# TinfoilHat0/Defending-Against-Backdoors-with-Robust-Learning-Rate

Measured on NVIDIA H100. Metric: fl_rounds_per_sec, higher is better.
Workload: dtype bf16

## Files before the change

defending-against-backdoors-with-robust-learning-rate_b200/ops/csrc/conv_halo.cu:

```cuda
#include <cuda.h>

#include "common.cuh"
#include "gemm.h"
#include "wgmma.cuh"

namespace rlr {

using namespace wg;

cudaError_t make_tmap_bf16(CUtensorMap* map, const void* base, int rank, const uint64_t* dims, const uint64_t* strides_bytes,
                           const uint32_t* box, const uint32_t* elem_strides = nullptr);

constexpr int HL_THREADS = 256 + 32;
constexpr int HL_TH = 16, HL_TW = 8;
constexpr int HL_PITCH = 16;
constexpr int HL_HALO_BYTES = (HL_TH + 2) * HL_PITCH * 128;
constexpr int HL_W_BYTES = 9 * 64 * 128;
constexpr int HL_STAGES = 3;
constexpr int HL_PITCH_OUT = 64 * 2 + 16;
constexpr int HL_STAGING = 128 * HL_PITCH_OUT;
constexpr int HL_SMEM = HL_W_BYTES + HL_STAGES * HL_HALO_BYTES + 2 * HL_STAGING + 1024 + 1024;

struct HaloParams {
    int NB, H, W;
// ... 104 lines not shown
                    const uint64_t db = smem_desc_sw128(w_base + tp * 8192 + k * 32, 16, 1024);
#pragma unroll
                    for (int m = 0; m < 2; ++m) {
                        const uint32_t a0 = halo + (dy * HL_PITCH + dx) * 128 + m * 8 * HL_PITCH * 128 + k * 32;
                        const uint32_t bo = p.bo_mode ? ((a0 >> 7) & 7u) : 0u;
                        wgmma_bf16<64, 0, 0>(acc[m], smem_desc_sw128(a0, 16, HL_PITCH * 128, bo), db, (tp > 0 || k > 0) ? 1u : 0u);
                    }
                }
            }
            wgmma_commit();
            wgmma_wait<0>();
            fence_acc(acc[0]);
            fence_acc(acc[1]);
            if (lane == 0) mbar_arrive(&sh->halo_empty[stage]);
            if (trace) p.dbg[q * 8 + 3] = clock64();
#pragma unroll
            for (int m = 0; m < 2; ++m)
#pragma unroll
                for (int j = 0; j < 8; ++j) {
                    const int c = frag_col(t, 4 * j);
#pragma unroll
                    for (int h = 0; h < 2; ++h) {
                        float a = acc[m][4 * j + 2 * h], b = acc[m][4 * j + 2 * h + 1];
                        a += sh->bias[c]; b += sh->bias[c + 1];
                        if (p.relu) { a = fmaxf(a, 0.f); b = fmaxf(b, 0.f); }
                        const uint32_t packed = pack_bf16x2(a, b);
                        if (kStats) {
                            const float2 rq = __bfloat1622float2(*reinterpret_cast<const __nv_bfloat162*>(&packed));
                            st1[2 * j] += rq.x; st1[2 * j + 1] += rq.y;
                            st2[2 * j] += rq.x * rq.x; st2[2 * j + 1] += rq.y * rq.y;
                        }
                        *reinterpret_cast<uint32_t*>(stage_buf + (m * 64 + r0 + 8 * h) * HL_PITCH_OUT + c * 2) = packed;
                    }
                }
            named_bar(1 + wgi, 128);
            if (trace) p.dbg[q * 8 + 6] = clock64();
#pragma unroll
            for (int it = 0; it < 8; ++it) {
                const int idx = t + it * 128;
                const int rr = idx >> 3, ch = idx & 7;
                if (col0 + ch * 8 >= p.N) continue;
                const int h = h0 + (rr >> 3), w = w0 + (rr & 7);
                if (h >= p.H || w >= p.W) continue;
                const size_t gi = ((size_t)n * p.H + h) * p.W + w;
                uint4 val = *reinterpret_cast<const uint4*>(stage_buf + rr * HL_PITCH_OUT + ch * 16);
                uint4* gp = reinterpret_cast<uint4*>(out + gi * p.ldc + col0 + ch * 8);
                if (kAcc) {
                    const __nv_bfloat162* o2 = reinterpret_cast<const __nv_bfloat162*>(&oldv[it]);
                    __nv_bfloat162* v2 = reinterpret_cast<__nv_bfloat162*>(&val);
#pragma unroll
                    for (int qq = 0; qq < 4; ++qq) {
                        const float2 a = __bfloat1622float2(v2[qq]), b = __bfloat1622float2(o2[qq]);
                        v2[qq] = __floats2bfloat162_rn(a.x + b.x, a.y + b.y);
                    }
                }
                *gp = val;
            }
            named_bar(1 + wgi, 128);
            if (trace) p.dbg[q * 8 + 7] = clock64();
        }
        if (kStats) {
#pragma unroll
            for (int i = 0; i < 16; ++i)
#pragma unroll
                for (int o = 4; o < 32; o <<= 1) {
                    st1[i] += __shfl_xor_sync(0xffffffffu, st1[i], o);
                    st2[i] += __shfl_xor_sync(0xffffffffu, st2[i], o);
                }
            if (lane < 4)
#pragma unroll
                for (int i = 0; i < 16; ++i) {
                    const int c = frag_col(t, 2 * (i & ~1)) + (i & 1);
                    atomicAdd(&sh->red[c], st1[i]);
                    atomicAdd(&sh->red[64 + c], st2[i]);
                }
            named_bar(3, 256);
            if (threadIdx.x < 128 && col0 + (threadIdx.x & 63) < p.N)
                atomicAdd(p.stats + (size_t)(blockIdx.x % kStatSlots) * 2 * p.N + (threadIdx.x < 64 ? 0 : p.N) + col0 + (threadIdx.x & 63),
                          sh->red[threadIdx.x]);
        }
    }
}

cudaError_t launch_conv3x3_halo_bf16(const void* x, const void* w, void* out, int NB, int Hin, int Win, int H, int W, int Cout, const float* bias,
                                     int relu, int accumulate, float* stats, int bo_mode, long long* dbg, int num_sms, cudaStream_t st) {
    const int pad = (H - Hin + 2) / 2;
    if (pad < 0 || pad > 2 || H != Hin + 2 * pad - 2 || W != Win + 2 * pad - 2 || H < 1 || W < 1 || Cout % 8) return cudaErrorInvalidValue;
    if (stats && (H % HL_TH || W % HL_TW)) return cudaErrorInvalidValue;
    static bool configured = false;
    if (!configured) {
        RLR_CUDA_CHECK(cudaFuncSetAttribute(umma_conv3x3_halo_kernel<false, false>, cudaFuncAttributeMaxDynamicSharedMemorySize, HL_SMEM));
        RLR_CUDA_CHECK(cudaFuncSetAttribute(umma_conv3x3_halo_kernel<true, false>, cudaFuncAttributeMaxDynamicSharedMemorySize, HL_SMEM));
        RLR_CUDA_CHECK(cudaFuncSetAttribute(umma_conv3x3_halo_kernel<false, true>, cudaFuncAttributeMaxDynamicSharedMemorySize, HL_SMEM));
        configured = true;
    }
    if (stats && accumulate) return cudaErrorInvalidValue;
    HaloParams p{};
    p.NB = NB; p.H = H; p.W = W; p.pad = pad;
    p.tiles_h = (H + HL_TH - 1) / HL_TH; p.tiles_w = (W + HL_TW - 1) / HL_TW; p.num_tiles = NB * p.tiles_h * p.tiles_w;
    p.N = Cout; p.out = out; p.ldc = Cout; p.bias = bias; p.stats = stats; p.relu = relu; p.accumulate = accumulate; p.bo_mode = bo_mode; p.dbg = dbg;
    CUtensorMap tmX, tmW;
    {
        const uint64_t d[4] = {64, (uint64_t)Win, (uint64_t)Hin, (uint64_t)NB};
        const uint64_t s[3] = {128, (uint64_t)Win * 128, (uint64_t)Hin * Win * 128};
        const uint32_t b[4] = {64, HL_PITCH, HL_TH + 2, 1};
        RLR_CUDA_CHECK(make_tmap_bf16(&tmX, x, 4, d, s, b));
    }
    {
        const uint64_t d[2] = {9 * 64, (uint64_t)Cout}, s[1] = {9 * 64 * 2};
        const uint32_t b[2] = {64, 64};
        RLR_CUDA_CHECK(make_tmap_bf16(&tmW, w, 2, d, s, b));
    }
    const int n_tiles_n = (Cout + 63) / 64;
    int gx = num_sms / n_tiles_n;
    if (gx > p.num_tiles) gx = p.num_tiles;
    if (gx < 1) gx = 1;
    const dim3 grid(gx, n_tiles_n);
    if (stats) return launch_kernel(umma_conv3x3_halo_kernel<true, false>, grid, dim3(HL_THREADS), HL_SMEM, st, tmX, tmW, p);
    if (accumulate) return launch_kernel(umma_conv3x3_halo_kernel<false, true>, grid, dim3(HL_THREADS), HL_SMEM, st, tmX, tmW, p);
    return launch_kernel(umma_conv3x3_halo_kernel<false, false>, grid, dim3(HL_THREADS), HL_SMEM, st, tmX, tmW, p);
}

}
```

defending-against-backdoors-with-robust-learning-rate_b200/ops/csrc/gemm.h:

```cpp
#pragma once
#include <cuda_runtime.h>
#include <cuda_bf16.h>
#include <stdint.h>

#include "dropspec.h"

namespace rlr {

constexpr int kStatSlots = 16;

struct ConvGemmParams {
    int M, N, num_kb;
    int mode;
    int cblocks;
    int TW, TH, TN;
    int Ho, Wo, NB;
    int tiles_w, tiles_h;
    int ntaps;
    int in_stride;
    int out_stride, out_ph, out_pw, OutH, OutW;
    int8_t dh[9], dw[9];
    int dn[9];
    int b_mn;
    int wtap[9];
    int wcols;
    DropSpec drop;
    int tma_store;
    int split_prod;
    long long* dbg;
    const __nv_bfloat16* b_src;
    int b_ld, b_kvalid;
    const uint32_t* wait_flags;
    int wait_lo, wait_hi;
    const uint32_t* wait_epoch;
    void* out;
    int ldc;
    const float* bias;
    float* stats;
    int stat_slots;
    int relu, accumulate;
};

cudaError_t launch_gemm_bf16(const void* A, const void* B, void* out, int M, int N, int K, int lda, int ldb, int ldc,
                             const float* bias, int relu, int accumulate, float* stats, cudaStream_t st, const DropSpec* drop = nullptr);
cudaError_t launch_stem_gemm_bf16(const void* A, const void* W, void* out, int M, int N, int kvalid, int ldw, const float* bias, int relu,
                                  float* stats, const uint32_t* wait_flags, int wait_lo, int wait_hi, const uint32_t* wait_epoch,
                                  cudaStream_t st);
void set_pdl(int on);
cudaError_t launch_gemm_splitk_bf16(const void* A, const void* B, void* out, float* ws, int M, int N, int K, const float* bias, int relu,
                                    int num_sms, cudaStream_t st, const DropSpec* drop = nullptr);
void set_persistent_conv(int on);
void set_conv_occ3(int level);
void set_conv_one_wave(int on);
void set_conv_tma_store(int on);
void set_conv_split_producer(int on);
void set_conv_trace(long long* buf);
long long* conv_trace_buf();
cudaError_t launch_conv_bf16(const void* x, const void* w, void* out, int NB, int planes, int Hin, int Win, int Cin, int Ho, int Wo,
                             int Cout, int ldc, int ntaps, const int* dh, const int* dw, const int* dplane, const float* bias,
                             int relu, int accumulate, float* stats, cudaStream_t st, const int* wtap = nullptr, int w_taps_total = 0,
                             int in_stride = 1, int out_stride = 1, int out_ph = 0, int out_pw = 0);

cudaError_t launch_conv3x3_halo_bf16(const void* x, const void* w, void* out, int NB, int Hin, int Win, int H, int W, int Cout, const float* bias,
                                     int relu, int accumulate, float* stats, int bo_mode, long long* dbg, int num_sms, cudaStream_t st);

cudaError_t launch_conv3x3_halo3_bf16(const void* x, const void* w, void* out, int NB, int H, int W, int Cout, const float* bias, int relu,
                                      int accumulate, int num_sms, cudaStream_t st);

cudaError_t launch_conv_wgrad_bf16(const void* dy, const void* x, float* dW, int NB, int planes, int Hin, int Win, int Cin, int Cin_valid,
                                   int Ho, int Wo, int Cout, int ntaps, const int* dh, const int* dw, const int* dplane, int num_sms,
                                   cudaStream_t st, int in_stride = 1);
cudaError_t launch_conv_wgrad_halo_bf16(const void* dy, const void* x, float* dW, int NB, int H, int W, int Cin_valid, int Cout,
                                        int num_sms, cudaStream_t st);
void set_wgrad_rows(int on);
void wgrad_launch_counts(long long* out);
cudaError_t launch_linear_wgrad_bf16(const void* dy, const void* x, float* dW, int B, int N, int K, int num_sms, cudaStream_t st);

cudaError_t launch_ordered_sum_f32(float* out, const float* part, int nparts, long long n, cudaStream_t st);
cudaError_t launch_ordered_sum_f64(double* out, const double* part, int nparts, long long n, cudaStream_t st);
cudaError_t launch_channel_stats(const __nv_bfloat16* x, long long M, int C, float* stats , int num_sms, cudaStream_t st,
                                 int only_sum = 0, int nslots = 1);
cudaError_t launch_bn_finalize(const float* stats, int slots, float* mean_rstd, float* running_mean, float* running_var, int C,
                               float count, float eps, float momentum, int train, cudaStream_t st);
cudaError_t launch_bn_apply(const __nv_bfloat16* x, const __nv_bfloat16* res, __nv_bfloat16* y, const float* gamma, const float* beta,
                            float* mean_rstd, long long M, int C, int relu, int fin_mode, const float* stats, int slots, float count,
                            float eps, float momentum, float* running_mean, float* running_var, int num_sms, cudaStream_t st);
cudaError_t launch_bn_bwd_reduce(const __nv_bfloat16* dy, const __nv_bfloat16* y, const __nv_bfloat16* x, const float* mean_rstd,
                                 float* dsum , long long M, int C, int relu, int num_sms, cudaStream_t st,
                                 const float* gamma = nullptr, const float* beta = nullptr, int nslots = 1);
cudaError_t launch_bn_bwd_apply(const __nv_bfloat16* dy, const __nv_bfloat16* y, const __nv_bfloat16* x, const float* gamma,
                                const float* mean_rstd, const float* dsum, __nv_bfloat16* dx, __nv_bfloat16* dres, float* dgamma,
                                float* dbeta, long long M, int C, int relu, int num_sms, cudaStream_t st, const float* beta = nullptr, int nslots = 1);
cudaError_t launch_gn_fwd(const __nv_bfloat16* x, const __nv_bfloat16* res, __nv_bfloat16* y, const float* gamma, const float* beta,
                          float* mean_rstd, int B, int HW, int C, int G, float eps, int relu, int num_sms, cudaStream_t st);
cudaError_t launch_gn_bwd(const __nv_bfloat16* dy, const __nv_bfloat16* y, const __nv_bfloat16* x, const float* gamma,
                          const float* mean_rstd, __nv_bfloat16* dx, __nv_bfloat16* dres, float* dgamma, float* dbeta, int B, int HW,
                          int C, int G, int relu, int num_sms, cudaStream_t st);
cudaError_t launch_relu_bwd(__nv_bfloat16* dy, const __nv_bfloat16* y, long long n, int num_sms, cudaStream_t st, float scale = 1.0f);
cudaError_t launch_maxpool2_fwd(const __nv_bfloat16* x, __nv_bfloat16* y, uint8_t* idx, int B, int H, int W, int C, cudaStream_t st,
                                float drop_p = 0.f, uint64_t seed = 0, const long long* step = nullptr, uint64_t stream = 0);
cudaError_t launch_maxpool2_bwd(const __nv_bfloat16* dy, const uint8_t* idx, __nv_bfloat16* dx, int B, int H, int W, int C, cudaStream_t st,
                                float drop_p, uint64_t seed, const long long* step, uint64_t stream, const __nv_bfloat16* zmask);
cudaError_t launch_avgpool_fwd(const __nv_bfloat16* x, __nv_bfloat16* y, int B, int HW, int C, cudaStream_t st);
cudaError_t launch_avgpool_bwd(const __nv_bfloat16* dy, __nv_bfloat16* dx, int B, int HW, int C, cudaStream_t st);
cudaError_t launch_dropout_fwd(const __nv_bfloat16* x, __nv_bfloat16* y, uint8_t* mask, long long n, float p, uint64_t seed,
                               const long long* step, uint64_t stream, cudaStream_t st);
cudaError_t launch_dropout_bwd(const __nv_bfloat16* dy, const uint8_t* mask, __nv_bfloat16* dx, long long n, float p, cudaStream_t st);
cudaError_t launch_space_to_depth(const __nv_bfloat16* x, __nv_bfloat16* y, int NB, int H, int W, int C, int num_sms, cudaStream_t st);
cudaError_t launch_im2col_small(const __nv_bfloat16* x, __nv_bfloat16* A, int NB, int H, int W, int C, int Ho, int Wo, int k, int pad,
                                int num_sms, cudaStream_t st);
cudaError_t launch_depth_to_space(const __nv_bfloat16* x4, __nv_bfloat16* y, int NB, int H, int W, int C, int accumulate, int plane_mask,
                                  int num_sms, cudaStream_t st);
cudaError_t launch_filter_gather_transpose(const __nv_bfloat16* w, __nv_bfloat16* wt, int Cout, int T, int Cin, int nsub, const int* taps,
                                           cudaStream_t st);
cudaError_t launch_filter_transpose(const __nv_bfloat16* w, __nv_bfloat16* wt, int Cout, int ntaps, int Cin, cudaStream_t st);
cudaError_t launch_linear_small_fwd(const __nv_bfloat16* x, const __nv_bfloat16* w, const float* bias, __nv_bfloat16* y, int B, int K,
                                    int N, int relu, cudaStream_t st);
cudaError_t launch_linear_small_fwd2(const __nv_bfloat16* x, const __nv_bfloat16* w, const float* bias, __nv_bfloat16* y, int B, int K,
                                     int N, int relu, cudaStream_t st);
cudaError_t launch_linear_small_bwd2(const __nv_bfloat16* x, const __nv_bfloat16* dy, const __nv_bfloat16* w, __nv_bfloat16* dx,
                                     float* dw, float* db, int B, int K, int N, int accumulate_dx, cudaStream_t st);
cudaError_t launch_linear_small_bwd(const __nv_bfloat16* x, const __nv_bfloat16* dy, const __nv_bfloat16* w, __nv_bfloat16* dx,
                                    float* dw, float* db, int B, int K, int N, int accumulate_dx, cudaStream_t st);

}
```

defending-against-backdoors-with-robust-learning-rate_b200/ops/csrc/gemm_binding.cpp:

```cpp
#include <torch/extension.h>
#include <ATen/cuda/CUDAContext.h>
#include <c10/cuda/CUDAGuard.h>
#include <c10/cuda/CUDAStream.h>
#include <c10/cuda/CUDACachingAllocator.h>

#include <vector>

#include "gemm.h"

namespace rlr {
void* scratch_alloc(size_t bytes, cudaStream_t st) {
    return c10::cuda::CUDACachingAllocator::raw_alloc_with_stream(bytes < 256 ? 256 : bytes, st);
}
void scratch_free(void* p) { c10::cuda::CUDACachingAllocator::raw_delete(p); }
}

namespace {
inline cudaStream_t cur_stream() { return c10::cuda::getCurrentCUDAStream().stream(); }
inline int num_sms() { return at::cuda::getCurrentDeviceProperties()->multiProcessorCount; }
inline void check(cudaError_t e, const char* what) { TORCH_CHECK(e == cudaSuccess, what, ": ", cudaGetErrorString(e)); }
template <typename T>
inline T* opt(const c10::optional<at::Tensor>& t) { return t.has_value() && t->defined() ? reinterpret_cast<T*>(t->data_ptr()) : nullptr; }
inline const __nv_bfloat16* bf(const at::Tensor& t) {
    TORCH_CHECK(t.is_cuda() && t.scalar_type() == at::kBFloat16 && t.is_contiguous(), "expected contiguous CUDA bf16 tensor");
// ... 255 lines not shown
void maxpool2_bwd(at::Tensor dy, at::Tensor idx, at::Tensor dx, double drop_p, int64_t drop_seed, c10::optional<at::Tensor> drop_step, int64_t drop_stream,
                  c10::optional<at::Tensor> relu_out) {
    c10::cuda::CUDAGuard g(dx.device());
    const rlr::DropSpec d = drop_spec(drop_p, drop_seed, drop_step, drop_stream);
    const bool zm = relu_out.has_value() && relu_out->defined();
    TORCH_CHECK(!zm || (relu_out->scalar_type() == at::kBFloat16 && relu_out->is_contiguous() && relu_out->numel() == dy.numel()), "relu_out must match dy");
    TORCH_CHECK(dy.is_contiguous() && dx.is_contiguous() && idx.is_contiguous() && dy.size(1) == dx.size(1) / 2 && dy.size(2) == dx.size(2) / 2);
    check(rlr::launch_maxpool2_bwd(bf(dy), (const uint8_t*)idx.data_ptr(), bfm(dx), dx.size(0), dx.size(1), dx.size(2), dx.size(3), cur_stream(),
                                   (float)drop_p, d.seed, d.step, d.stream, zm ? bf(*relu_out) : nullptr), "maxpool2_bwd");
}
void avgpool_fwd(at::Tensor x, at::Tensor y) {
    c10::cuda::CUDAGuard g(x.device());
    check(rlr::launch_avgpool_fwd(bf(x), bfm(y), x.size(0), x.size(1) * x.size(2), x.size(3), cur_stream()), "avgpool_fwd");
}
void avgpool_bwd(at::Tensor dy, at::Tensor dx) {
    c10::cuda::CUDAGuard g(dx.device());
    check(rlr::launch_avgpool_bwd(bf(dy), bfm(dx), dx.size(0), dx.size(1) * dx.size(2), dx.size(3), cur_stream()), "avgpool_bwd");
}
void dropout_fwd(at::Tensor x, at::Tensor y, at::Tensor mask, double p, int64_t seed, at::Tensor step, int64_t stream) {
    c10::cuda::CUDAGuard g(x.device());
    check(rlr::launch_dropout_fwd(bf(x), bfm(y), (uint8_t*)mask.data_ptr(), x.numel(), (float)p, (uint64_t)seed,
                                  (const long long*)step.data_ptr(), (uint64_t)stream, cur_stream()), "dropout_fwd");
}
void dropout_bwd(at::Tensor dy, at::Tensor mask, at::Tensor dx, double p) {
    c10::cuda::CUDAGuard g(dx.device());
    check(rlr::launch_dropout_bwd(bf(dy), (const uint8_t*)mask.data_ptr(), bfm(dx), dx.numel(), (float)p, cur_stream()), "dropout_bwd");
}
void space_to_depth(at::Tensor x, at::Tensor y) {
    c10::cuda::CUDAGuard g(x.device());
    check(rlr::launch_space_to_depth(bf(x), bfm(y), x.size(0), x.size(1), x.size(2), x.size(3), num_sms(), cur_stream()), "space_to_depth");
}
void im2col_small(at::Tensor x, at::Tensor A, int64_t k, int64_t pad) {
    c10::cuda::CUDAGuard g(x.device());
    const int NB = x.size(0), H = x.size(1), W = x.size(2), C = x.size(3);
    const int Ho = H + 2 * pad - k + 1, Wo = W + 2 * pad - k + 1;
    TORCH_CHECK(x.dim() == 4 && x.is_contiguous() && A.is_contiguous() && A.numel() == (int64_t)NB * Ho * Wo * 64, "im2col_small: A must be [NB*Ho*Wo, 64]");
    check(rlr::launch_im2col_small(bf(x), bfm(A), NB, H, W, C, Ho, Wo, (int)k, (int)pad, num_sms(), cur_stream()), "im2col_small");
}
void depth_to_space(at::Tensor x4, at::Tensor y, bool accumulate, int64_t plane_mask) {
    c10::cuda::CUDAGuard g(y.device());
    check(rlr::launch_depth_to_space(bf(x4), bfm(y), y.size(0), y.size(1), y.size(2), y.size(3), accumulate, (int)plane_mask, num_sms(),
                                     cur_stream()), "depth_to_space");
}
void filter_gather_transpose(at::Tensor w, at::Tensor wt, int64_t Cout, int64_t T, int64_t Cin, std::vector<int64_t> taps) {
    c10::cuda::CUDAGuard g(w.device());
    int t[9];
    TORCH_CHECK(taps.size() >= 1 && taps.size() <= 9);
    for (size_t i = 0; i < taps.size(); ++i) t[i] = (int)taps[i];
    check(rlr::launch_filter_gather_transpose(bf(w), bfm(wt), Cout, T, Cin, (int)taps.size(), t, cur_stream()), "filter_gather_transpose");
}
void filter_transpose(at::Tensor w, at::Tensor wt, int64_t Cout, int64_t ntaps, int64_t Cin) {
    c10::cuda::CUDAGuard g(w.device());
    check(rlr::launch_filter_transpose(bf(w), bfm(wt), Cout, ntaps, Cin, cur_stream()), "filter_transpose");
}
void linear_small_fwd(at::Tensor x, at::Tensor w, c10::optional<at::Tensor> bias, at::Tensor y, bool relu) {
    c10::cuda::CUDAGuard g(x.device());
    check(rlr::launch_linear_small_fwd(bf(x), bf(w), opt<const float>(bias), bfm(y), x.size(0), x.size(1), w.size(0), relu, cur_stream()), "linear_small_fwd");
}
void linear_small_bwd(at::Tensor x, at::Tensor dy, at::Tensor w, c10::optional<at::Tensor> dx, at::Tensor dw, c10::optional<at::Tensor> db,
                      bool accumulate_dx) {
    c10::cuda::CUDAGuard g(x.device());
    check(rlr::launch_linear_small_bwd(bf(x), bf(dy), bf(w), const_cast<__nv_bfloat16*>(bfo(dx)), (float*)dw.data_ptr(), opt<float>(db),
                                       x.size(0), x.size(1), w.size(0), accumulate_dx, cur_stream()), "linear_small_bwd");
}
void linear_small_fwd2(at::Tensor x, at::Tensor w, c10::optional<at::Tensor> bias, at::Tensor y, bool relu) {
    c10::cuda::CUDAGuard g(x.device());
    check(rlr::launch_linear_small_fwd2(bf(x), bf(w), opt<const float>(bias), bfm(y), x.size(0), x.size(1), w.size(0), relu, cur_stream()), "linear_small_fwd2");
}
void linear_small_bwd2(at::Tensor x, at::Tensor dy, at::Tensor w, c10::optional<at::Tensor> dx, at::Tensor dw, c10::optional<at::Tensor> db,
                       bool accumulate_dx) {
    c10::cuda::CUDAGuard g(x.device());
    check(rlr::launch_linear_small_bwd2(bf(x), bf(dy), bf(w), const_cast<__nv_bfloat16*>(bfo(dx)), (float*)dw.data_ptr(), opt<float>(db),
                                        x.size(0), x.size(1), w.size(0), accumulate_dx, cur_stream()), "linear_small_bwd2");
}
}

void register_gemm_bindings(py::module_& m) {
    m.attr("STAT_SLOTS") = rlr::kStatSlots;
    m.def("set_persistent_conv", [](bool on) { rlr::set_persistent_conv(on ? 1 : 0); });
    m.def("set_pdl", [](bool on) { rlr::set_pdl(on ? 1 : 0); });
    m.def("set_conv_occ3", [](int64_t level) { rlr::set_conv_occ3((int)level); });
    m.def("set_conv_one_wave", [](bool on) { rlr::set_conv_one_wave(on ? 1 : 0); });
    m.def("set_wgrad_rows", [](bool on) { rlr::set_wgrad_rows(on ? 1 : 0); });
    m.def("wgrad_launch_counts", [] {
        long long c[3];
        rlr::wgrad_launch_counts(c);
        return std::vector<int64_t>{c[0], c[1], c[2]};
    });
    m.def("set_conv_tma_store", [](bool on) { rlr::set_conv_tma_store(on ? 1 : 0); });
    m.def("set_conv_split_producer", [](bool on) { rlr::set_conv_split_producer(on ? 1 : 0); });
    m.def("set_conv_trace", [](c10::optional<at::Tensor> buf) {
        rlr::set_conv_trace(buf.has_value() && buf->defined() ? reinterpret_cast<long long*>(buf->data_ptr<int64_t>()) : nullptr);
    });
    m.def("gemm_bf16", &gemm_bf16, py::arg("A"), py::arg("B"), py::arg("out"), py::arg("bias"), py::arg("relu"), py::arg("accumulate"), py::arg("stats"),
          py::arg("drop_p") = 0.0, py::arg("drop_seed") = 0, py::arg("drop_step") = py::none(), py::arg("drop_stream") = 0);
    m.def("stem_gemm_bf16", &stem_gemm_bf16, py::arg("A"), py::arg("W"), py::arg("out"), py::arg("bias"), py::arg("relu"), py::arg("stats"),
          py::arg("ready_ptr") = 0, py::arg("lo") = 0, py::arg("hi") = 0, py::arg("epoch") = py::none());
    m.def("gemm_splitk_bf16", &gemm_splitk_bf16, py::arg("A"), py::arg("B"), py::arg("out"), py::arg("ws"), py::arg("bias"), py::arg("relu"),
          py::arg("drop_p") = 0.0, py::arg("drop_seed") = 0, py::arg("drop_step") = py::none(), py::arg("drop_stream") = 0);
    m.def("conv_bf16", &conv_bf16);
    m.def("conv_bf16_strided", &conv_bf16_strided);
    m.def("conv_wgrad_bf16_strided", &conv_wgrad_bf16_strided);
    m.def("conv3x3_halo_bf16", &conv3x3_halo_bf16);
    m.def("conv3x3_halo3_bf16", &conv3x3_halo3_bf16);
    m.def("conv_wgrad_bf16", &conv_wgrad_bf16);
    m.def("linear_wgrad_bf16", &linear_wgrad_bf16);
    m.def("conv_wgrad_halo_bf16", &conv_wgrad_halo_bf16);
    m.def("channel_stats", &channel_stats);
    m.def("ordered_sum", &ordered_sum);
    m.def("bias_grad", &bias_grad);
    m.def("bn_finalize", &bn_finalize);
    m.def("bn_apply", &bn_apply);
    m.def("bn_bwd", &bn_bwd);
    m.def("bn_bwd_recompute", &bn_bwd_recompute);
    m.def("gn_fwd", &gn_fwd);
    m.def("gn_bwd", &gn_bwd);
    m.def("relu_bwd", &relu_bwd, py::arg("dy"), py::arg("y"), py::arg("scale") = 1.0);
    m.def("maxpool2_fwd", &maxpool2_fwd, py::arg("x"), py::arg("y"), py::arg("idx"), py::arg("drop_p") = 0.0, py::arg("drop_seed") = 0,
          py::arg("drop_step") = py::none(), py::arg("drop_stream") = 0);
    m.def("maxpool2_bwd", &maxpool2_bwd, py::arg("dy"), py::arg("idx"), py::arg("dx"), py::arg("drop_p") = 0.0, py::arg("drop_seed") = 0,
          py::arg("drop_step") = py::none(), py::arg("drop_stream") = 0, py::arg("relu_out") = py::none());
    m.def("avgpool_fwd", &avgpool_fwd);
    m.def("avgpool_bwd", &avgpool_bwd);
    m.def("dropout_fwd", &dropout_fwd);
    m.def("dropout_bwd", &dropout_bwd);
    m.def("space_to_depth", &space_to_depth);
    m.def("im2col_small", &im2col_small);
    m.def("filter_transpose", &filter_transpose);
    m.def("depth_to_space", &depth_to_space);
    m.def("filter_gather_transpose", &filter_gather_transpose);
    m.def("linear_small_fwd", &linear_small_fwd);
    m.def("linear_small_bwd", &linear_small_bwd);
    m.def("linear_small_fwd2", &linear_small_fwd2);
    m.def("linear_small_bwd2", &linear_small_bwd2);
}
```

defending-against-backdoors-with-robust-learning-rate_b200/ops/csrc/wgmma.cuh:

```cuda
#pragma once
#include <cuda.h>
#include <cuda_runtime.h>
#include <stdint.h>

namespace rlr {
namespace wg {

__device__ __forceinline__ uint32_t smem_u32(const void* p) { return (uint32_t)__cvta_generic_to_shared(p); }

__device__ __forceinline__ void mbar_init(uint64_t* bar, uint32_t count) {
    asm volatile("mbarrier.init.shared::cta.b64 [%0], %1;" ::"r"(smem_u32(bar)), "r"(count) : "memory");
}
__device__ __forceinline__ void fence_barrier_init() { asm volatile("fence.mbarrier_init.release.cluster;" ::: "memory"); }
__device__ __forceinline__ void mbar_expect_tx(uint64_t* bar, uint32_t bytes) {
    asm volatile("mbarrier.arrive.expect_tx.shared::cta.b64 _, [%0], %1;" ::"r"(smem_u32(bar)), "r"(bytes) : "memory");
}
__device__ __forceinline__ void mbar_arrive(uint64_t* bar) {
    asm volatile("mbarrier.arrive.shared::cta.b64 _, [%0];" ::"r"(smem_u32(bar)) : "memory");
}
__device__ __forceinline__ void mbar_wait(uint64_t* bar, uint32_t parity) {
    const uint32_t addr = smem_u32(bar);
    asm volatile(
        "{\n\t"
        ".reg .pred P1;\n\t"
        "WAIT_LOOP:\n\t"
        "mbarrier.try_wait.parity.shared::cta.b64 P1, [%0], %1;\n\t"
        "@P1 bra WAIT_DONE;\n\t"
        "bra WAIT_LOOP;\n\t"
        "WAIT_DONE:\n\t"
        "}\n" ::"r"(addr), "r"(parity) : "memory");
}

__device__ __forceinline__ void prefetch_tmap(const CUtensorMap* m) {
    asm volatile("prefetch.tensormap [%0];" ::"l"(reinterpret_cast<uint64_t>(m)) : "memory");
}
__device__ __forceinline__ void tma_load_2d(const CUtensorMap* m, uint64_t* bar, void* dst, int c0, int c1) {
    asm volatile("cp.async.bulk.tensor.2d.shared::cluster.global.mbarrier::complete_tx::bytes [%0], [%1, {%3, %4}], [%2];"
                 ::"r"(smem_u32(dst)), "l"(reinterpret_cast<uint64_t>(m)), "r"(smem_u32(bar)), "r"(c0), "r"(c1) : "memory");
}
__device__ __forceinline__ void tma_load_4d(const CUtensorMap* m, uint64_t* bar, void* dst, int c0, int c1, int c2, int c3) {
    asm volatile("cp.async.bulk.tensor.4d.shared::cluster.global.mbarrier::complete_tx::bytes [%0], [%1, {%3, %4, %5, %6}], [%2];"
                 ::"r"(smem_u32(dst)), "l"(reinterpret_cast<uint64_t>(m)), "r"(smem_u32(bar)), "r"(c0), "r"(c1), "r"(c2), "r"(c3)
                 : "memory");
}

__device__ __forceinline__ void tma_store_2d(const CUtensorMap* m, const void* src, int c0, int c1) {
    asm volatile("cp.async.bulk.tensor.2d.global.shared::cta.bulk_group [%0, {%2, %3}], [%1];"
                 ::"l"(reinterpret_cast<uint64_t>(m)), "r"(smem_u32(src)), "r"(c0), "r"(c1) : "memory");
}
__device__ __forceinline__ void tma_store_4d(const CUtensorMap* m, const void* src, int c0, int c1, int c2, int c3) {
    asm volatile("cp.async.bulk.tensor.4d.global.shared::cta.bulk_group [%0, {%2, %3, %4, %5}], [%1];"
                 ::"l"(reinterpret_cast<uint64_t>(m)), "r"(smem_u32(src)), "r"(c0), "r"(c1), "r"(c2), "r"(c3) : "memory");
}
__device__ __forceinline__ void tma_store_commit() { asm volatile("cp.async.bulk.commit_group;" ::: "memory"); }
__device__ __forceinline__ void tma_store_wait_read() { asm volatile("cp.async.bulk.wait_group.read 0;" ::: "memory"); }
__device__ __forceinline__ void fence_proxy_async_smem() { asm volatile("fence.proxy.async.shared::cta;" ::: "memory"); }

__device__ __forceinline__ void named_bar(int id, int threads) { asm volatile("bar.sync %0, %1;" ::"r"(id), "r"(threads) : "memory"); }

__device__ __forceinline__ uint64_t smem_desc_sw128(uint32_t saddr, uint32_t lbo_bytes, uint32_t sbo_bytes, uint32_t base_offset = 0) {
    return (uint64_t)((saddr >> 4) & 0x3FFFu) | ((uint64_t)((lbo_bytes >> 4) & 0x3FFFu) << 16) |
           ((uint64_t)((sbo_bytes >> 4) & 0x3FFFu) << 32) | ((uint64_t)(base_offset & 7u) << 49) | (1ull << 62);
}

__device__ __forceinline__ void wgmma_fence() { asm volatile("wgmma.fence.sync.aligned;" ::: "memory"); }
__device__ __forceinline__ void wgmma_commit() { asm volatile("wgmma.commit_group.sync.aligned;" ::: "memory"); }
template <int kPending>
__device__ __forceinline__ void wgmma_wait() { asm volatile("wgmma.wait_group.sync.aligned %0;" ::"n"(kPending) : "memory"); }
template <int R>
__device__ __forceinline__ void fence_acc(float (&d)[R]) {
#pragma unroll
    for (int i = 0; i < R; ++i) asm volatile("" : "+f"(d[i])::"memory");
}

template <int kTransA, int kTransB>
__device__ __forceinline__ void wgmma_m64n64(float (&d)[32], uint64_t desc_a, uint64_t desc_b, uint32_t accumulate) {
    asm volatile(
        "{\n\t.reg .pred p;\n\tsetp.ne.b32 p, %34, 0;\n\t"
        "wgmma.mma_async.sync.aligned.m64n64k16.f32.bf16.bf16 {%0, %1, %2, %3, %4, %5, %6, %7, %8, %9, %10, %11, %12, %13, %14, %15, %16, %17, %18, %19, %20, %21, %22, %23, %24, %25, %26, %27, %28, %29, %30, %31}, %32, %33, p, 1, 1, %35, %36;\n\t}\n"
        : "+f"(d[0]), "+f"(d[1]), "+f"(d[2]), "+f"(d[3]), "+f"(d[4]), "+f"(d[5]), "+f"(d[6]), "+f"(d[7]), "+f"(d[8]), "+f"(d[9]), "+f"(d[10]), "+f"(d[11]), "+f"(d[12]), "+f"(d[13]), "+f"(d[14]), "+f"(d[15]), "+f"(d[16]), "+f"(d[17]), "+f"(d[18]), "+f"(d[19]), "+f"(d[20]), "+f"(d[21]), "+f"(d[22]), "+f"(d[23]), "+f"(d[24]), "+f"(d[25]), "+f"(d[26]), "+f"(d[27]), "+f"(d[28]), "+f"(d[29]), "+f"(d[30]), "+f"(d[31])
        : "l"(desc_a), "l"(desc_b), "r"(accumulate), "n"(kTransA), "n"(kTransB));
}
template <int kTransA, int kTransB>
__device__ __forceinline__ void wgmma_m64n128(float (&d)[64], uint64_t desc_a, uint64_t desc_b, uint32_t accumulate) {
    asm volatile(
        "{\n\t.reg .pred p;\n\tsetp.ne.b32 p, %66, 0;\n\t"
        "wgmma.mma_async.sync.aligned.m64n128k16.f32.bf16.bf16 {%0, %1, %2, %3, %4, %5, %6, %7, %8, %9, %10, %11, %12, %13, %14, %15, %16, %17, %18, %19, %20, %21, %22, %23, %24, %25, %26, %27, %28, %29, %30, %31, %32, %33, %34, %35, %36, %37, %38, %39, %40, %41, %42, %43, %44, %45, %46, %47, %48, %49, %50, %51, %52, %53, %54, %55, %56, %57, %58, %59, %60, %61, %62, %63}, %64, %65, p, 1, 1, %67, %68;\n\t}\n"
        : "+f"(d[0]), "+f"(d[1]), "+f"(d[2]), "+f"(d[3]), "+f"(d[4]), "+f"(d[5]), "+f"(d[6]), "+f"(d[7]), "+f"(d[8]), "+f"(d[9]), "+f"(d[10]), "+f"(d[11]), "+f"(d[12]), "+f"(d[13]), "+f"(d[14]), "+f"(d[15]), "+f"(d[16]), "+f"(d[17]), "+f"(d[18]), "+f"(d[19]), "+f"(d[20]), "+f"(d[21]), "+f"(d[22]), "+f"(d[23]), "+f"(d[24]), "+f"(d[25]), "+f"(d[26]), "+f"(d[27]), "+f"(d[28]), "+f"(d[29]), "+f"(d[30]), "+f"(d[31]), "+f"(d[32]), "+f"(d[33]), "+f"(d[34]), "+f"(d[35]), "+f"(d[36]), "+f"(d[37]), "+f"(d[38]), "+f"(d[39]), "+f"(d[40]), "+f"(d[41]), "+f"(d[42]), "+f"(d[43]), "+f"(d[44]), "+f"(d[45]), "+f"(d[46]), "+f"(d[47]), "+f"(d[48]), "+f"(d[49]), "+f"(d[50]), "+f"(d[51]), "+f"(d[52]), "+f"(d[53]), "+f"(d[54]), "+f"(d[55]), "+f"(d[56]), "+f"(d[57]), "+f"(d[58]), "+f"(d[59]), "+f"(d[60]), "+f"(d[61]), "+f"(d[62]), "+f"(d[63])
        : "l"(desc_a), "l"(desc_b), "r"(accumulate), "n"(kTransA), "n"(kTransB));
}
template <int kTransA, int kTransB>
__device__ __forceinline__ void wgmma_m64n192(float (&d)[96], uint64_t desc_a, uint64_t desc_b, uint32_t accumulate) {
    asm volatile(
        "{\n\t.reg .pred p;\n\tsetp.ne.b32 p, %98, 0;\n\t"
        "wgmma.mma_async.sync.aligned.m64n192k16.f32.bf16.bf16 {%0, %1, %2, %3, %4, %5, %6, %7, %8, %9, %10, %11, %12, %13, %14, %15, %16, %17, %18, %19, %20, %21, %22, %23, %24, %25, %26, %27, %28, %29, %30, %31, %32, %33, %34, %35, %36, %37, %38, %39, %40, %41, %42, %43, %44, %45, %46, %47, %48, %49, %50, %51, %52, %53, %54, %55, %56, %57, %58, %59, %60, %61, %62, %63, %64, %65, %66, %67, %68, %69, %70, %71, %72, %73, %74, %75, %76, %77, %78, %79, %80, %81, %82, %83, %84, %85, %86, %87, %88, %89, %90, %91, %92, %93, %94, %95}, %96, %97, p, 1, 1, %99, %100;\n\t}\n"
        : "+f"(d[0]), "+f"(d[1]), "+f"(d[2]), "+f"(d[3]), "+f"(d[4]), "+f"(d[5]), "+f"(d[6]), "+f"(d[7]), "+f"(d[8]), "+f"(d[9]), "+f"(d[10]), "+f"(d[11]), "+f"(d[12]), "+f"(d[13]), "+f"(d[14]), "+f"(d[15]), "+f"(d[16]), "+f"(d[17]), "+f"(d[18]), "+f"(d[19]), "+f"(d[20]), "+f"(d[21]), "+f"(d[22]), "+f"(d[23]), "+f"(d[24]), "+f"(d[25]), "+f"(d[26]), "+f"(d[27]), "+f"(d[28]), "+f"(d[29]), "+f"(d[30]), "+f"(d[31]), "+f"(d[32]), "+f"(d[33]), "+f"(d[34]), "+f"(d[35]), "+f"(d[36]), "+f"(d[37]), "+f"(d[38]), "+f"(d[39]), "+f"(d[40]), "+f"(d[41]), "+f"(d[42]), "+f"(d[43]), "+f"(d[44]), "+f"(d[45]), "+f"(d[46]), "+f"(d[47]), "+f"(d[48]), "+f"(d[49]), "+f"(d[50]), "+f"(d[51]), "+f"(d[52]), "+f"(d[53]), "+f"(d[54]), "+f"(d[55]), "+f"(d[56]), "+f"(d[57]), "+f"(d[58]), "+f"(d[59]), "+f"(d[60]), "+f"(d[61]), "+f"(d[62]), "+f"(d[63]), "+f"(d[64]), "+f"(d[65]), "+f"(d[66]), "+f"(d[67]), "+f"(d[68]), "+f"(d[69]), "+f"(d[70]), "+f"(d[71]), "+f"(d[72]), "+f"(d[73]), "+f"(d[74]), "+f"(d[75]), "+f"(d[76]), "+f"(d[77]), "+f"(d[78]), "+f"(d[79]), "+f"(d[80]), "+f"(d[81]), "+f"(d[82]), "+f"(d[83]), "+f"(d[84]), "+f"(d[85]), "+f"(d[86]), "+f"(d[87]), "+f"(d[88]), "+f"(d[89]), "+f"(d[90]), "+f"(d[91]), "+f"(d[92]), "+f"(d[93]), "+f"(d[94]), "+f"(d[95])
        : "l"(desc_a), "l"(desc_b), "r"(accumulate), "n"(kTransA), "n"(kTransB));
}

template <int N, int kTransA, int kTransB>
__device__ __forceinline__ void wgmma_bf16(float (&d)[N / 2], uint64_t desc_a, uint64_t desc_b, uint32_t accumulate) {
    if constexpr (N == 64) wgmma_m64n64<kTransA, kTransB>(d, desc_a, desc_b, accumulate);
    else if constexpr (N == 128) wgmma_m64n128<kTransA, kTransB>(d, desc_a, desc_b, accumulate);
    else wgmma_m64n192<kTransA, kTransB>(d, desc_a, desc_b, accumulate);
}

__device__ __forceinline__ int frag_row(int t, int i) { return ((t >> 5) << 4) + ((t & 31) >> 2) + (((i >> 1) & 1) << 3); }
__device__ __forceinline__ int frag_col(int t, int i) { return ((i >> 2) << 3) + ((t & 3) << 1) + (i & 1); }

template <int BN, int kStages, int kStageBytes, int kABytes, bool kBMN>
__device__ __forceinline__ void consumer_mainloop(float (&acc)[BN / 2], uint8_t* smem, uint64_t* full, uint64_t* empty, int num_kb,
                                                  uint32_t a_off, uint32_t b_fixed, int& stage, uint32_t& phase, int lane) {
    int prev = -1;
    for (int kb = 0; kb < num_kb; ++kb) {
        mbar_wait(&full[stage], phase);
        const uint32_t sa = smem_u32(smem + stage * kStageBytes);
        const uint32_t sb = b_fixed ? b_fixed : sa + kABytes;
        wgmma_fence();
#pragma unroll
        for (int k = 0; k < 4; ++k) {
            const uint64_t da = smem_desc_sw128(sa + a_off + k * 32, 16, 1024);
            const uint64_t db = kBMN ? smem_desc_sw128(sb + k * 2048, 8192, 1024) : smem_desc_sw128(sb + k * 32, 16, 1024);
            wgmma_bf16<BN, 0, kBMN ? 1 : 0>(acc, da, db, (kb > 0 || k > 0) ? 1u : 0u);
        }
        wgmma_commit();
        wgmma_wait<1>();
        if (prev >= 0 && lane == 0) mbar_arrive(&empty[prev]);
        prev = stage;
        if (++stage == kStages) { stage = 0; phase ^= 1; }
    }
    wgmma_wait<0>();
    fence_acc(acc);
    if (prev >= 0 && lane == 0) mbar_arrive(&empty[prev]);
}

}
}
```

Measured before the change: 0.7314.

## Add transposed-operand halo conv kernel using wgmma N=128 and stmatrix epilogue

Adds a new 3x3 halo convolution kernel that swaps the GEMM operands: weights become the A operand (64 output channels as M) and the 128 spatial positions of the halo tile become the B operand, so each wgmma is m64n128 rather than m64n64. The epilogue transposes the accumulator through stmatrix.trans into a staging buffer before writing coalesced 16-byte stores, and the per-channel stats reduction is simplified because each thread now owns only two channels. The new path is on by default behind a runtime flag. It aims to cut wgmma instruction count and epilogue reduction overhead, but relies on the B-operand descriptor addressing the halo layout correctly and adds register pressure from 64 accumulators plus the prefetched accumulate values.

```diff
diff --git a/defending-against-backdoors-with-robust-learning-rate_b200/ops/csrc/conv_halo.cu b/defending-against-backdoors-with-robust-learning-rate_b200/ops/csrc/conv_halo.cu
--- a/defending-against-backdoors-with-robust-learning-rate_b200/ops/csrc/conv_halo.cu
+++ b/defending-against-backdoors-with-robust-learning-rate_b200/ops/csrc/conv_halo.cu
@@ -210,6 +210,169 @@
     }
 }
 
+template <bool kStats, bool kAcc>
+__global__ void __launch_bounds__(HL_THREADS, 1)
+umma_conv3x3_halo_t_kernel(const __grid_constant__ CUtensorMap tmX, const __grid_constant__ CUtensorMap tmW, const HaloParams p) {
+    extern __shared__ uint8_t smem_raw[];
+    uint8_t* smem = reinterpret_cast<uint8_t*>((reinterpret_cast<uintptr_t>(smem_raw) + 1023) & ~uintptr_t(1023));
+    uint8_t* s_w = smem;
+    uint8_t* s_halo = smem + HL_W_BYTES;
+    uint8_t* s_stage = s_halo + HL_STAGES * HL_HALO_BYTES;
+    HaloShared* sh = reinterpret_cast<HaloShared*>(s_stage + 2 * HL_STAGING);
+    const int warp = threadIdx.x >> 5, lane = threadIdx.x & 31;
+    const int tile_n = blockIdx.y;
+    const int col0 = tile_n * 64;
+
+    if (warp == 8 && lane == 0) {
+        prefetch_tmap(&tmX); prefetch_tmap(&tmW);
+        mbar_init(&sh->w_full, 1);
+        for (int s = 0; s < HL_STAGES; ++s) { mbar_init(&sh->halo_full[s], 1); mbar_init(&sh->halo_empty[s], 4); }
+        fence_barrier_init();
+    }
+    if (threadIdx.x < 128) sh->red[threadIdx.x] = 0.f;
+    const int tiles_per_img = p.tiles_h * p.tiles_w;
+    pdl_wait();
+    pdl_trigger();
+    if (threadIdx.x < 64) sh->bias[threadIdx.x] = (p.bias && col0 + (int)threadIdx.x < p.N) ? p.bias[col0 + threadIdx.x] : 0.f;
+    __syncthreads();
+
+    if (warp == 8) {
+        if (lane == 0) {
+            mbar_expect_tx(&sh->w_full, HL_W_BYTES);
+            for (int t = 0; t < 9; ++t) tma_load_2d(&tmW, &sh->w_full, s_w + t * 8192, t * 64, tile_n * 64);
+            int stage = 0;
+            uint32_t phase = 0;
+            for (int tile = blockIdx.x; tile < p.num_tiles; tile += gridDim.x) {
+                const int n = tile / tiles_per_img, r = tile - n * tiles_per_img;
+                const int h0 = (r / p.tiles_w) * HL_TH, w0 = (r % p.tiles_w) * HL_TW;
+                mbar_wait(&sh->halo_empty[stage], phase ^ 1);
+                mbar_expect_tx(&sh->halo_full[stage], HL_HALO_BYTES);
+                tma_load_4d(&tmX, &sh->halo_full[stage], s_halo + stage * HL_HALO_BYTES, 0, w0 - p.pad, h0 - p.pad, n);
+                if (++stage == HL_STAGES) { stage = 0; phase ^= 1; }
+            }
+        }
+    } else {
+        const int wgi = threadIdx.x >> 7, t = threadIdx.x & 127;
+        uint8_t* stage_buf = s_stage + wgi * HL_STAGING;
+        const int co0 = frag_row(t, 0);
+        const float bias0 = sh->bias[co0], bias1 = sh->bias[co0 + 8];
+        const uint32_t st_base = smem_u32(stage_buf) + (8 * (lane >> 4) + (lane & 7)) * HL_PITCH_OUT + (16 * (t >> 5) + 8 * ((lane >> 3) & 1)) * 2;
+        __nv_bfloat16* out = reinterpret_cast<__nv_bfloat16*>(p.out);
+        float st1[2] = {0.f, 0.f}, st2[2] = {0.f, 0.f};
+        const uint32_t w_base = smem_u32(s_w);
+        mbar_wait(&sh->w_full, 0);
+        for (int q = wgi;; q += 2) {
+            const int tile = blockIdx.x + q * gridDim.x;
+            if (tile >= p.num_tiles) break;
+            const int stage = q % HL_STAGES;
+            const uint32_t phase = (uint32_t)(q / HL_STAGES) & 1u;
+            const int n = tile / tiles_per_img, r = tile - n * tiles_per_img;
+            const int h0 = (r / p.tiles_w) * HL_TH, w0 = (r % p.tiles_w) * HL_TW;
+            uint4 oldv[8];
+            if (kAcc) {
+#pragma unroll
+                for (int it = 0; it < 8; ++it) {
+                    const int idx = t + it * 128, rr = idx >> 3, ch = idx & 7;
+                    const int h = h0 + (rr >> 3), w = w0 + (rr & 7);
+                    oldv[it] = make_uint4(0, 0, 0, 0);
+                    if (col0 + ch * 8 < p.N && h < p.H && w < p.W)
+                        oldv[it] = *reinterpret_cast<const uint4*>(out + (((size_t)n * p.H + h) * p.W + w) * p.ldc + col0 + ch * 8);
+                }
+            }
+            const bool trace = p.dbg && blockIdx.x == 0 && blockIdx.y == 0 && t == 0;
+            if (trace) p.dbg[q * 8 + 0] = clock64();
+            mbar_wait(&sh->halo_full[stage], phase);
+            if (trace) p.dbg[q * 8 + 2] = clock64();
+            const uint32_t halo = smem_u32(s_halo + stage * HL_HALO_BYTES);
+            float acc[64];
+#pragma unroll
+            for (int i = 0; i < 64; ++i) acc[i] = 0.f;
+            wgmma_fence();
+#pragma unroll
+            for (int tp = 0; tp < 9; ++tp) {
+                const int dy = tp / 3, dx = tp - dy * 3;
+#pragma unroll
+                for (int k = 0; k < 4; ++k) {
+                    const uint64_t da = smem_desc_sw128(w_base + tp * 8192 + k * 32, 16, 1024);
+                    const uint32_t b0 = halo + (dy * HL_PITCH + dx) * 128 + k * 32;
+                    const uint32_t bo = p.bo_mode ? ((b0 >> 7) & 7u) : 0u;
+                    wgmma_bf16<128, 0, 0>(acc, da, smem_desc_sw128(b0, 16, HL_PITCH * 128, bo), (tp > 0 || k > 0) ? 1u : 0u);
+                }
+            }
+            wgmma_commit();
+            wgmma_wait<0>();
+            fence_acc(acc);
+            if (lane == 0) mbar_arrive(&sh->halo_empty[stage]);
+            if (trace) p.dbg[q * 8 + 3] = clock64();
+#pragma unroll
+            for (int jj = 0; jj < 8; ++jj) {
+                uint32_t frag[4];
+#pragma unroll
+                for (int i = 0; i < 4; ++i) {
+                    const int j = 2 * jj + (i >> 1), h = i & 1;
+                    float a = acc[4 * j + 2 * h], b = acc[4 * j + 2 * h + 1];
+                    a += h ? bias1 : bias0; b += h ? bias1 : bias0;
+                    if (p.relu) { a = fmaxf(a, 0.f); b = fmaxf(b, 0.f); }
+                    frag[i] = pack_bf16x2(a, b);
+                    if (kStats) {
+                        const float2 rq = __bfloat1622float2(*reinterpret_cast<const __nv_bfloat162*>(&frag[i]));
+                        st1[h] += rq.x + rq.y;
+                        st2[h] += rq.x * rq.x + rq.y * rq.y;
+                    }
+                }
+                stmatrix_x4_trans(st_base + 16 * jj * HL_PITCH_OUT, frag);
+            }
+            named_bar(1 + wgi, 128);
+            if (trace) p.dbg[q * 8 + 6] = clock64();
+#pragma unroll
+            for (int it = 0; it < 8; ++it) {
+                const int idx = t + it * 128;
+                const int rr = idx >> 3, ch = idx & 7;
+                if (col0 + ch * 8 >= p.N) continue;
+                const int h = h0 + (rr >> 3), w = w0 + (rr & 7);
+                if (h >= p.H || w >= p.W) continue;
+                const size_t gi = ((size_t)n * p.H + h) * p.W + w;
+                uint4 val = *reinterpret_cast<const uint4*>(stage_buf + rr * HL_PITCH_OUT + ch * 16);
+                uint4* gp = reinterpret_cast<uint4*>(out + gi * p.ldc + col0 + ch * 8);
+                if (kAcc) {
+                    const __nv_bfloat162* o2 = reinterpret_cast<const __nv_bfloat162*>(&oldv[it]);
+                    __nv_bfloat162* v2 = reinterpret_cast<__nv_bfloat162*>(&val);
+#pragma unroll
+                    for (int qq = 0; qq < 4; ++qq) {
+                        const float2 a = __bfloat1622float2(v2[qq]), b = __bfloat1622float2(o2[qq]);
+                        v2[qq] = __floats2bfloat162_rn(a.x + b.x, a.y + b.y);
+                    }
+                }
+                *gp = val;
+            }
+            named_bar(1 + wgi, 128);
+            if (trace) p.dbg[q * 8 + 7] = clock64();
+        }
+        if (kStats) {
+#pragma unroll
+            for (int h = 0; h < 2; ++h)
+#pragma unroll
+                for (int o = 1; o < 4; o <<= 1) {
+                    st1[h] += __shfl_xor_sync(0xffffffffu, st1[h], o);
+                    st2[h] += __shfl_xor_sync(0xffffffffu, st2[h], o);
+                }
+            if ((lane & 3) == 0)
+#pragma unroll
+                for (int h = 0; h < 2; ++h) {
+                    atomicAdd(&sh->red[co0 + 8 * h], st1[h]);
+                    atomicAdd(&sh->red[64 + co0 + 8 * h], st2[h]);
+                }
+            named_bar(3, 256);
+            if (threadIdx.x < 128 && col0 + (threadIdx.x & 63) < p.N)
+                atomicAdd(p.stats + (size_t)(blockIdx.x % kStatSlots) * 2 * p.N + (threadIdx.x < 64 ? 0 : p.N) + col0 + (threadIdx.x & 63),
+                          sh->red[threadIdx.x]);
+        }
+    }
+}
+
+static int g_halo_swap = 1;
+void set_conv_halo_swap(int on) { g_halo_swap = on ? 1 : 0; }
+
 cudaError_t launch_conv3x3_halo_bf16(const void* x, const void* w, void* out, int NB, int Hin, int Win, int H, int W, int Cout, const float* bias,
                                      int relu, int accumulate, float* stats, int bo_mode, long long* dbg, int num_sms, cudaStream_t st) {
     const int pad = (H - Hin + 2) / 2;
@@ -220,6 +383,9 @@
         RLR_CUDA_CHECK(cudaFuncSetAttribute(umma_conv3x3_halo_kernel<false, false>, cudaFuncAttributeMaxDynamicSharedMemorySize, HL_SMEM));
         RLR_CUDA_CHECK(cudaFuncSetAttribute(umma_conv3x3_halo_kernel<true, false>, cudaFuncAttributeMaxDynamicSharedMemorySize, HL_SMEM));
         RLR_CUDA_CHECK(cudaFuncSetAttribute(umma_conv3x3_halo_kernel<false, true>, cudaFuncAttributeMaxDynamicSharedMemorySize, HL_SMEM));
+        RLR_CUDA_CHECK(cudaFuncSetAttribute(umma_conv3x3_halo_t_kernel<false, false>, cudaFuncAttributeMaxDynamicSharedMemorySize, HL_SMEM));
+        RLR_CUDA_CHECK(cudaFuncSetAttribute(umma_conv3x3_halo_t_kernel<true, false>, cudaFuncAttributeMaxDynamicSharedMemorySize, HL_SMEM));
+        RLR_CUDA_CHECK(cudaFuncSetAttribute(umma_conv3x3_halo_t_kernel<false, true>, cudaFuncAttributeMaxDynamicSharedMemorySize, HL_SMEM));
         configured = true;
     }
     if (stats && accumulate) return cudaErrorInvalidValue;
@@ -244,6 +410,11 @@
     if (gx > p.num_tiles) gx = p.num_tiles;
     if (gx < 1) gx = 1;
     const dim3 grid(gx, n_tiles_n);
+    if (g_halo_swap) {
+        if (stats) return launch_kernel(umma_conv3x3_halo_t_kernel<true, false>, grid, dim3(HL_THREADS), HL_SMEM, st, tmX, tmW, p);
+        if (accumulate) return launch_kernel(umma_conv3x3_halo_t_kernel<false, true>, grid, dim3(HL_THREADS), HL_SMEM, st, tmX, tmW, p);
+        return launch_kernel(umma_conv3x3_halo_t_kernel<false, false>, grid, dim3(HL_THREADS), HL_SMEM, st, tmX, tmW, p);
+    }
     if (stats) return launch_kernel(umma_conv3x3_halo_kernel<true, false>, grid, dim3(HL_THREADS), HL_SMEM, st, tmX, tmW, p);
     if (accumulate) return launch_kernel(umma_conv3x3_halo_kernel<false, true>, grid, dim3(HL_THREADS), HL_SMEM, st, tmX, tmW, p);
     return launch_kernel(umma_conv3x3_halo_kernel<false, false>, grid, dim3(HL_THREADS), HL_SMEM, st, tmX, tmW, p);
diff --git a/defending-against-backdoors-with-robust-learning-rate_b200/ops/csrc/gemm.h b/defending-against-backdoors-with-robust-learning-rate_b200/ops/csrc/gemm.h
--- a/defending-against-backdoors-with-robust-learning-rate_b200/ops/csrc/gemm.h
+++ b/defending-against-backdoors-with-robust-learning-rate_b200/ops/csrc/gemm.h
@@ -63,6 +63,7 @@
 
 cudaError_t launch_conv3x3_halo_bf16(const void* x, const void* w, void* out, int NB, int Hin, int Win, int H, int W, int Cout, const float* bias,
                                      int relu, int accumulate, float* stats, int bo_mode, long long* dbg, int num_sms, cudaStream_t st);
+void set_conv_halo_swap(int on);
 
 cudaError_t launch_conv3x3_halo3_bf16(const void* x, const void* w, void* out, int NB, int H, int W, int Cout, const float* bias, int relu,
                                       int accumulate, int num_sms, cudaStream_t st);
diff --git a/defending-against-backdoors-with-robust-learning-rate_b200/ops/csrc/gemm_binding.cpp b/defending-against-backdoors-with-robust-learning-rate_b200/ops/csrc/gemm_binding.cpp
--- a/defending-against-backdoors-with-robust-learning-rate_b200/ops/csrc/gemm_binding.cpp
+++ b/defending-against-backdoors-with-robust-learning-rate_b200/ops/csrc/gemm_binding.cpp
@@ -361,6 +361,7 @@
     m.def("set_conv_occ3", [](int64_t level) { rlr::set_conv_occ3((int)level); });
     m.def("set_conv_one_wave", [](bool on) { rlr::set_conv_one_wave(on ? 1 : 0); });
     m.def("set_wgrad_rows", [](bool on) { rlr::set_wgrad_rows(on ? 1 : 0); });
+    m.def("set_conv_halo_swap", [](bool on) { rlr::set_conv_halo_swap(on ? 1 : 0); });
     m.def("wgrad_launch_counts", [] {
         long long c[3];
         rlr::wgrad_launch_counts(c);
diff --git a/defending-against-backdoors-with-robust-learning-rate_b200/ops/csrc/wgmma.cuh b/defending-against-backdoors-with-robust-learning-rate_b200/ops/csrc/wgmma.cuh
--- a/defending-against-backdoors-with-robust-learning-rate_b200/ops/csrc/wgmma.cuh
+++ b/defending-against-backdoors-with-robust-learning-rate_b200/ops/csrc/wgmma.cuh
@@ -57,6 +57,11 @@
 __device__ __forceinline__ void fence_proxy_async_smem() { asm volatile("fence.proxy.async.shared::cta;" ::: "memory"); }
 
 __device__ __forceinline__ void named_bar(int id, int threads) { asm volatile("bar.sync %0, %1;" ::"r"(id), "r"(threads) : "memory"); }
+
+__device__ __forceinline__ void stmatrix_x4_trans(uint32_t saddr, const uint32_t (&r)[4]) {
+    asm volatile("stmatrix.sync.aligned.m8n8.x4.trans.shared.b16 [%0], {%1, %2, %3, %4};"
+                 ::"r"(saddr), "r"(r[0]), "r"(r[1]), "r"(r[2]), "r"(r[3]) : "memory");
+}
 
 __device__ __forceinline__ uint64_t smem_desc_sw128(uint32_t saddr, uint32_t lbo_bytes, uint32_t sbo_bytes, uint32_t base_offset = 0) {
     return (uint64_t)((saddr >> 4) & 0x3FFFu) | ((uint64_t)((lbo_bytes >> 4) & 0x3FFFu) << 16) |
```

Result: faster. 0.7454, median of 6 (+1.9%).
